# uber-research/UPSNet

Hardware: NVIDIA H100
Metric: panoptic images/sec at 1024x2048 (higher is better)
Workload: dtype bf16x3

## Files before the change

### upsnet_b200/csrc/dcn_win.cu

```cuda
#include <cuda.h>
#include <cuda_bf16.h>

#include "common.cuh"
#include "tc_ptx.cuh"
#include "tc_params.cuh"

namespace ups {

constexpr int DW_BM = 128;
constexpr int DW_WW = 32, DW_WH = 20;
constexpr int DW_PLANE = DW_WW * DW_WH * 32;
constexpr int DW_WIN_BYTES = 2 * DW_PLANE;
constexpr int DW_WIN_BUFS = 2;
constexpr int DW_KHW = 9;
constexpr int DW_GROUPS = 2;
constexpr int DW_EPI_PITCH = 36;
constexpr uint32_t DW_EPI_BYTES = DW_BM * DW_EPI_PITCH * 4;

constexpr uint32_t DW_OFF_BARS = 0;
constexpr uint32_t DW_OFF_STATS = 192;
constexpr uint32_t DW_OFF_ORG = 256;
constexpr uint32_t DW_OFF_TW = 512;
constexpr uint32_t DW_OFF_TP = DW_OFF_TW + DW_KHW * DW_BM * 16;
constexpr uint32_t DW_OFF_STAGES = DW_OFF_TP + DW_KHW * DW_BM * 4;
static_assert(DW_OFF_STAGES % 1024 == 0, "stage buffers need 1024-byte alignment (SWIZZLE_128B)");

template <int BN> struct DwCfg {
  static constexpr int NCW = BN == 128 ? 2 : 1;
  static constexpr int FRAGS = 2 / NCW;
  static constexpr int BK = BN == 128 ? 32 : 64;
  static constexpr int SPK = BK / 16;
  static constexpr int ROWB = BK * 2;
  static constexpr int CONSUMERS = 128 * NCW;
  static constexpr int WARP_TMAB = CONSUMERS / 32, WARP_TMAW = WARP_TMAB + 1, WARP_PROD0 = WARP_TMAB + 4;
  static constexpr int GROUP = 4 * (SPK / 2) * 32;
  static constexpr int PRODUCERS = GROUP * DW_GROUPS;
  static constexpr int THREADS = WARP_PROD0 * 32 + PRODUCERS;
  static constexpr int WARPGROUPS = THREADS / 128;
  static constexpr int REGS_LAUNCH = 16384 / (32 * ((THREADS / 32 + 3) / 4)) / 8 * 8;
  static constexpr int REGS_TMA = 32, REGS_CONSUMER = 128;
  static_assert(NCW * REGS_CONSUMER + REGS_TMA + (PRODUCERS / 128) * REGS_LAUNCH <= WARPGROUPS * REGS_LAUNCH,
                "setmaxnreg budgets exceed the CTA's register allocation");
  static constexpr int TABLE_IT = (DW_KHW * DW_BM + PRODUCERS - 1) / PRODUCERS;
  static constexpr uint32_t A_BYTES = 2 * DW_BM * ROWB;
  static constexpr uint32_t B_BYTES = BN * ROWB;
  static constexpr uint32_t STAGE_BYTES = 2 * B_BYTES + A_BYTES;
  static_assert(STAGE_BYTES % 1024 == 0, "stages must keep the 1024-byte alignment of the swizzled tiles");
  static constexpr int STAGES = BN == 128 ? 3 : 2;
  static_assert(STAGES <= 3, "the barrier map holds three stages");
  static constexpr uint32_t OFF_WIN = DW_OFF_STAGES + STAGES * STAGE_BYTES;
  static constexpr uint32_t OFF_EPI = OFF_WIN + DW_WIN_BUFS * DW_WIN_BYTES;
  static constexpr uint32_t SMEM = OFF_EPI + DW_EPI_BYTES + 1024;
  static_assert(SMEM <= 227 * 1024, "shared memory exceeds 227 KB");
};
template <int ROWB> __device__ __forceinline__ uint32_t dw_chunk(uint32_t j, uint32_t r) {
  return ROWB == 128 ? (j ^ (r & 7u)) : (j ^ ((r >> 1) & 3u));
}

struct DwParams {
  const void* x;
  const float* offset;
  const float* mask;
  const float* bias;
  void* y;
  int N, H, W, Cin, Cout, Cout_pad, Ho, Wo, ph, pw, dh, dw, relu, BN, tile_w, tile_h;
};

template <int BN>
__global__ void __launch_bounds__(DwCfg<BN>::THREADS, 1)
dcn_win_kernel(const __grid_constant__ CUtensorMap tm_x, const __grid_constant__ CUtensorMap tm_w, const __grid_constant__ DwParams p) {
  using C = DwCfg<BN>;
  constexpr int DW_PRODUCERS = C::PRODUCERS, DW_CONSUMERS = C::CONSUMERS;
  constexpr int DW_WARP_TMAB = C::WARP_TMAB, DW_WARP_TMAW = C::WARP_TMAW, DW_WARP_PROD0 = C::WARP_PROD0;
  constexpr int DW_BK = C::BK, SPK = C::SPK, ROWB = C::ROWB;
  extern __shared__ __align__(1024) uint8_t smem_dyn[];
  const uint32_t raw = smem_u32(smem_dyn);
  const uint32_t base = (raw + 1023u) & ~1023u;
  uint8_t* sm = smem_dyn + (base - raw);

  const int tid = threadIdx.x, warp = tid >> 5, lane = tid & 31;
  const uint32_t b_bytes = C::B_BYTES;
  const uint32_t stage_bytes = C::STAGE_BYTES;
  constexpr uint32_t NST = C::STAGES, NWB = DW_WIN_BUFS;
  const uint32_t win_base = base + C::OFF_WIN;
  float* stf = reinterpret_cast<float*>(sm + C::OFF_EPI);
  const uint32_t bar_fa = base + DW_OFF_BARS;
  const uint32_t bar_fb = bar_fa + 24;
  const uint32_t bar_em = bar_fa + 48;
  const uint32_t bar_wf = bar_fa + 104;
  const uint32_t bar_we = bar_fa + 120;
  const uint32_t bar_og = bar_fa + 136;
  int* stats = reinterpret_cast<int*>(sm + DW_OFF_STATS);
  int4* org = reinterpret_cast<int4*>(sm + DW_OFF_ORG);
  float4* tw = reinterpret_cast<float4*>(sm + DW_OFF_TW);
  int* tp = reinterpret_cast<int*>(sm + DW_OFF_TP);

  const int HoWo = p.Ho * p.Wo;
  const int nsc = p.Cin / 16;
  const int num_kb = nsc * DW_KHW / SPK;
  const int n_tiles = p.Cout_pad / BN;
  const int TW = p.tile_w, TH = p.tile_h;
  const int tw_shift = TW == 16 ? 4 : 3;
  const int tiles_w = (p.Wo + TW - 1) / TW, tiles_h = (p.Ho + TH - 1) / TH;
  const long long num_tiles = (long long)p.N * tiles_w * tiles_h * n_tiles;

  if (warp == 0) {
    if (lane == 0) {
      for (int s = 0; s < C::STAGES; ++s) {
        mbar_init(bar_fa + 8 * s, C::GROUP / 32);
        mbar_init(bar_fb + 8 * s, 1);
        mbar_init(bar_em + 8 * s, DW_CONSUMERS / 32);
      }
      for (int s = 0; s < 2; ++s) {
        mbar_init(bar_wf + 8 * s, 1);
        mbar_init(bar_we + 8 * s, DW_PRODUCERS / 32);
        mbar_init(bar_og + 8 * s, 1);
      }
      fence_mbar_init();
      for (int i = 0; i < 2; ++i) {
        stats[i * 8 + 0] = 0x7fffffff; stats[i * 8 + 1] = 0x7fffffff;
        stats[i * 8 + 2] = -0x7fffffff; stats[i * 8 + 3] = -0x7fffffff;
        stats[i * 8 + 4] = 0; stats[i * 8 + 5] = 0; stats[i * 8 + 6] = 0; stats[i * 8 + 7] = 0;
      }
    }
    __syncwarp();
  }
  if (warp == DW_WARP_TMAB && lane == 0) prefetch_tmap(&tm_w);
  if (warp == DW_WARP_TMAW && lane == 0) prefetch_tmap(&tm_x);
  __syncthreads();

  if (warp >= DW_WARP_PROD0) {
    const int pt = tid - DW_WARP_PROD0 * 32;
    const int pw = warp - DW_WARP_PROD0;
    const int group = pw / (C::GROUP / 32);
    const int u = (pw >> 2) & (SPK / 2 - 1);
    const int quad = pw & 3;
    const int r = quad * 32 + lane;
    const __nv_bfloat16* xh = reinterpret_cast<const __nv_bfloat16*>(p.x);
    uint32_t g0 = 0, wf0 = 0;
    uint32_t wf_ready = 0;
    uint32_t tile_it = 0;
    for (long long tile = blockIdx.x; tile < num_tiles; tile += gridDim.x, ++tile_it) {
      const long long mt = tile / n_tiles;
      const int tx = (int)(mt % tiles_w), ty = (int)((mt / tiles_w) % tiles_h), n = (int)(mt / ((long long)tiles_w * tiles_h));
      const int par = (int)(tile_it & 1u);
      constexpr int TIT = C::TABLE_IT;
      float4 ewv[TIT];
      int ehl[TIT], ewl[TIT];
      bool evalid[TIT];
      int mnw = 0x7fffffff, mnh = 0x7fffffff, mxw = -0x7fffffff, mxh = -0x7fffffff, sw_ = 0, sh_ = 0, cnt = 0;
#pragma unroll
      for (int it = 0; it < TIT; ++it) {
        const int e = pt + it * DW_PRODUCERS;
        ewv[it] = make_float4(0.f, 0.f, 0.f, 0.f);
        ehl[it] = 0; ewl[it] = 0; evalid[it] = false;
        if (e < DW_KHW * DW_BM) {
          const int tap = e >> 7, rr = e & 127;
          const int ry = rr >> tw_shift;
          const int wo = tx * TW + (rr & (TW - 1)), ho = ty * TH + ry;
          if (ry < TH && wo < p.Wo && ho < p.Ho) {
            const int pp = ho * p.Wo + wo;
            const int ki = tap / 3, kj = tap - ki * 3;
            const float* offp = p.offset + ((size_t)n * 2 * DW_KHW + 2 * tap) * HoWo + pp;
            const float oh = __ldg(offp), ow = __ldg(offp + HoWo);
            const float h = (float)(ho - p.ph + ki * p.dh) + oh;
            const float w = (float)(wo - p.pw + kj * p.dw) + ow;
            if (h > -1.f && w > -1.f && h < (float)p.H && w < (float)p.W) {
              const int hl = (int)floorf(h), wl = (int)floorf(w), hh = hl + 1, wh = wl + 1;
              const float lh = h - hl, lw = w - wl, ch = 1.f - lh, cw = 1.f - lw;
              const bool t_ok = hl >= 0, b_ok = hh <= p.H - 1, l_ok = wl >= 0, r_ok = wh <= p.W - 1;
              float m = 1.f;
              if (p.mask) m = __ldg(p.mask + ((size_t)n * DW_KHW + tap) * HoWo + pp);
              ewv[it].x = (t_ok && l_ok) ? ch * cw * m : 0.f;
              ewv[it].y = (t_ok && r_ok) ? ch * lw * m : 0.f;
              ewv[it].z = (b_ok && l_ok) ? lh * cw * m : 0.f;
              ewv[it].w = (b_ok && r_ok) ? lh * lw * m : 0.f;
              ehl[it] = hl; ewl[it] = wl; evalid[it] = true;
              mnw = min(mnw, wl); mxw = max(mxw, wl + 1); mnh = min(mnh, hl); mxh = max(mxh, hl + 1);
              sw_ += wl; sh_ += hl; ++cnt;
            }
          }
        }
      }
      mnw = __reduce_min_sync(0xffffffffu, mnw); mnh = __reduce_min_sync(0xffffffffu, mnh);
      mxw = __reduce_max_sync(0xffffffffu, mxw); mxh = __reduce_max_sync(0xffffffffu, mxh);
      sw_ = __reduce_add_sync(0xffffffffu, sw_); sh_ = __reduce_add_sync(0xffffffffu, sh_);
      cnt = __reduce_add_sync(0xffffffffu, cnt);
      if (lane == 0 && cnt > 0) {
        int* st = stats + par * 8;
        atomicMin(st + 0, mnw); atomicMin(st + 1, mnh); atomicMax(st + 2, mxw); atomicMax(st + 3, mxh);
        atomicAdd(st + 4, sw_); atomicAdd(st + 5, sh_); atomicAdd(st + 6, cnt);
      }
      named_bar<1, DW_PRODUCERS>();
      int ox = 0, oy = 0;
      {
        const int* st = stats + par * 8;
        const int c = st[6];
        if (c > 0) {
          const int a = st[0], b = st[1], cc = st[2], d = st[3];
          ox = (cc - a + 1 <= DW_WW) ? a : (int)floorf((float)st[4] / (float)c + 1.0f) - DW_WW / 2;
          oy = (d - b + 1 <= DW_WH) ? b : (int)floorf((float)st[5] / (float)c + 1.0f) - DW_WH / 2;
        }
      }
#pragma unroll
      for (int it = 0; it < TIT; ++it) {
        const int e = pt + it * DW_PRODUCERS;
        if (e < DW_KHW * DW_BM) {
          int code = 0;
          if (evalid[it]) {
            const int dx = ewl[it] - ox, dy = ehl[it] - oy;
            if (dx >= 0 && dx + 1 < DW_WW && dy >= 0 && dy + 1 < DW_WH) code = (dy * DW_WW + dx) * 32;
            else code = (int)(0x80000000u | ((uint32_t)(ehl[it] + 1) << 15) | (uint32_t)(ewl[it] + 1));
          }
          tw[e] = ewv[it];
          tp[e] = code;
        }
      }
      if (pt == 0) {
        org[par] = make_int4(ox, oy, n, 0);
        int* so = stats + (par ^ 1) * 8;
        so[0] = 0x7fffffff; so[1] = 0x7fffffff; so[2] = -0x7fffffff; so[3] = -0x7fffffff; so[4] = 0; so[5] = 0; so[6] = 0;
        mbar_arrive(bar_og + 8 * par);
      }
      named_bar<1, DW_PRODUCERS>();
      const __nv_bfloat16* ximg = xh + (size_t)n * p.H * p.W * (size_t)(2 * p.Cin);

      int rel = 0;
      for (int kb = (int)((uint32_t)(group - (int)g0) & 1u); kb < num_kb; kb += DW_GROUPS) {
        const uint32_t g = g0 + (uint32_t)kb;
        const uint32_t s = g % NST, it = g / NST;
        mbar_wait(bar_em + 8 * s, (it & 1u) ^ 1u);
        const uint32_t a_row = base + DW_OFF_STAGES + s * stage_bytes + 2 * b_bytes + (uint32_t)r * (uint32_t)ROWB;
#pragma unroll 1
        for (int pass = 0; pass < 4; ++pass) {
          const int sl = 2 * u + (pass >> 1), half = pass & 1;
          const int q = kb * SPK + sl;
          const int sc = q / DW_KHW, tap = q - sc * DW_KHW;
          const uint32_t wf = wf0 + (uint32_t)sc;
          if (wf >= wf_ready) {
            mbar_wait(bar_wf + 8 * (wf % NWB), (wf / NWB) & 1u);
            wf_ready = wf + 1;
          }
          const uint32_t wbuf = win_base + (wf % NWB) * (uint32_t)DW_WIN_BYTES;
          const int code = tp[tap * DW_BM + r];
          const uint32_t a_off = dw_chunk<ROWB>((uint32_t)(sl * 2 + half), (uint32_t)r) << 4;
          const float4 wv = tw[tap * DW_BM + r];
          uint4 hc[4], lc[4];
          if (code >= 0) {
            const uint32_t cl = (uint32_t)code, cr = cl + 32u;
            const uint32_t al = wbuf + cl + ((((cl >> 7) & 1u) ^ (uint32_t)half) << 4);
            const uint32_t ar = wbuf + cr + ((((cr >> 7) & 1u) ^ (uint32_t)half) << 4);
            hc[0] = lds128(al); hc[1] = lds128(ar); hc[2] = lds128(al + DW_WW * 32); hc[3] = lds128(ar + DW_WW * 32);
            lc[0] = lds128(al + DW_PLANE); lc[1] = lds128(ar + DW_PLANE);
            lc[2] = lds128(al + DW_PLANE + DW_WW * 32); lc[3] = lds128(ar + DW_PLANE + DW_WW * 32);
          } else {
            const int hl = (int)(((uint32_t)code >> 15) & 0xffffu) - 1, wl = (int)((uint32_t)code & 0x7fffu) - 1;
            const int h0 = max(hl, 0), h1 = min(hl + 1, p.H - 1), w0 = max(wl, 0), w1 = min(wl + 1, p.W - 1);
            const size_t pc = (size_t)(2 * p.Cin);
            const int cg = sc * 16 + half * 8;
            const __nv_bfloat16* b00 = ximg + ((size_t)h0 * p.W + w0) * pc + cg;
            const __nv_bfloat16* b01 = ximg + ((size_t)h0 * p.W + w1) * pc + cg;
            const __nv_bfloat16* b10 = ximg + ((size_t)h1 * p.W + w0) * pc + cg;
            const __nv_bfloat16* b11 = ximg + ((size_t)h1 * p.W + w1) * pc + cg;
            hc[0] = __ldg(reinterpret_cast<const uint4*>(b00)); lc[0] = __ldg(reinterpret_cast<const uint4*>(b00 + p.Cin));
            hc[1] = __ldg(reinterpret_cast<const uint4*>(b01)); lc[1] = __ldg(reinterpret_cast<const uint4*>(b01 + p.Cin));
            hc[2] = __ldg(reinterpret_cast<const uint4*>(b10)); lc[2] = __ldg(reinterpret_cast<const uint4*>(b10 + p.Cin));
            hc[3] = __ldg(reinterpret_cast<const uint4*>(b11)); lc[3] = __ldg(reinterpret_cast<const uint4*>(b11 + p.Cin));
          }
          uint4 ohi, olo;
          pair_blend8(wv, hc, lc, ohi, olo);
          sts128(a_row + a_off, ohi);
          sts128(a_row + DW_BM * ROWB + a_off, olo);
        }
        fence_proxy_async();
        __syncwarp();
        if (lane == 0) {
          mbar_arrive(bar_fa + 8 * s);
          while (rel < nsc && DW_KHW * (rel + 1) <= SPK * (kb + DW_GROUPS)) {
            mbar_arrive(bar_we + 8 * ((wf0 + (uint32_t)rel) % NWB));
            ++rel;
          }
        }
        rel = __shfl_sync(0xffffffffu, rel, 0);
      }
      if (lane == 0) {
        while (rel < nsc) { mbar_arrive(bar_we + 8 * ((wf0 + (uint32_t)rel) % NWB)); ++rel; }
      }
      __syncwarp();
      g0 += (uint32_t)num_kb;
      wf0 += (uint32_t)nsc;
    }
  } else if (warp >= DW_WARP_TMAB) {
    setmaxnreg_dec<C::REGS_TMA>();
    if (warp == DW_WARP_TMAW && lane == 0) {
      uint32_t wf = 0, ti = 0;
      for (long long tile = blockIdx.x; tile < num_tiles; tile += gridDim.x, ++ti) {
        const uint32_t par = ti & 1u;
        mbar_wait(bar_og + 8 * par, (ti >> 1) & 1u);
        const volatile int* ov = reinterpret_cast<const volatile int*>(&org[par]);
        const int4 o = make_int4(ov[0], ov[1], ov[2], 0);
        for (int f = 0; f < nsc; ++f, ++wf) {
          const uint32_t b = wf % NWB;
          mbar_wait(bar_we + 8 * b, ((wf / NWB) & 1u) ^ 1u);
          mbar_arrive_expect_tx(bar_wf + 8 * b, (uint32_t)DW_WIN_BYTES);
          const uint32_t dst = win_base + b * (uint32_t)DW_WIN_BYTES;
          tma_load_4d(dst, &tm_x, bar_wf + 8 * b, f * 16, o.x, o.y, o.z);
          tma_load_4d(dst + (uint32_t)DW_PLANE, &tm_x, bar_wf + 8 * b, p.Cin + f * 16, o.x, o.y, o.z);
        }
      }
    } else if (warp == DW_WARP_TMAB && lane == 0) {
      uint32_t g = 0;
      for (long long tile = blockIdx.x; tile < num_tiles; tile += gridDim.x) {
        const int n0 = (int)(tile % n_tiles) * BN;
        for (int kb = 0; kb < num_kb; ++kb, ++g) {
          const uint32_t s = g % NST, it = g / NST;
          mbar_wait(bar_em + 8 * s, (it & 1u) ^ 1u);
          const uint32_t stage = base + DW_OFF_STAGES + s * stage_bytes;
          mbar_arrive_expect_tx(bar_fb + 8 * s, 2 * b_bytes);
          tma_load_2d(stage, &tm_w, bar_fb + 8 * s, kb * DW_BK, n0);
          tma_load_2d(stage + b_bytes, &tm_w, bar_fb + 8 * s, kb * DW_BK, p.Cout_pad + n0);
        }
      }
    }
    __syncwarp();
  } else {
    setmaxnreg_inc<C::REGS_CONSUMER>();
    constexpr int FRAGS = C::FRAGS;
    const int wg = warp >> 2;
    const uint32_t dhi = ROWB == 128 ? wg_desc_hi(8 * ROWB) : wg_desc_hi_sw64(8 * ROWB);
    float d[FRAGS][BN / 2];
    constexpr uint32_t h16 = 64u * ROWB / 16u;
    __nv_bfloat16* yb = reinterpret_cast<__nv_bfloat16*>(p.y);
    uint32_t s = 0, ph = 0;
    for (long long tile = blockIdx.x; tile < num_tiles; tile += gridDim.x) {
      const long long mt = tile / n_tiles;
      const int n0 = (int)(tile % n_tiles) * BN;
      const int tx = (int)(mt % tiles_w), ty = (int)((mt / tiles_w) % tiles_h), n = (int)(mt / ((long long)tiles_w * tiles_h));
      int prev = -1;
      for (int kb = 0; kb < num_kb; ++kb) {
        mbar_wait(bar_fb + 8 * s, ph);
        mbar_wait(bar_fa + 8 * s, ph);
        const uint32_t st0 = base + DW_OFF_STAGES + s * stage_bytes;
        const uint32_t b_hi = wg_desc_lo(st0), b_lo = wg_desc_lo(st0 + b_bytes);
        const uint32_t a_hi = wg_desc_lo(st0 + 2 * b_bytes) + (uint32_t)(wg * FRAGS) * h16;
        const uint32_t a_lo = wg_desc_lo(st0 + 2 * b_bytes + DW_BM * ROWB) + (uint32_t)(wg * FRAGS) * h16;
        wgmma_fence();
#pragma unroll
        for (uint32_t k = 0; k < SPK; ++k) {
          const uint32_t acc = (kb | k) ? 1u : 0u;
          const uint64_t bh = wg_desc(b_hi + 2 * k, dhi), bl = wg_desc(b_lo + 2 * k, dhi);
#pragma unroll
          for (int f = 0; f < FRAGS; ++f) Wgmma<BN>::mma(d[f], wg_desc(a_lo + f * h16 + 2 * k, dhi), bh, acc);
#pragma unroll
          for (int f = 0; f < FRAGS; ++f) Wgmma<BN>::mma(d[f], wg_desc(a_hi + f * h16 + 2 * k, dhi), bl, 1u);
#pragma unroll
          for (int f = 0; f < FRAGS; ++f) Wgmma<BN>::mma(d[f], wg_desc(a_hi + f * h16 + 2 * k, dhi), bh, 1u);
        }
        wgmma_commit();
        wgmma_wait<1>();
#pragma unroll
        for (int f = 0; f < FRAGS; ++f) wgmma_fence_acc(d[f]);
        if (prev >= 0 && lane == 0) mbar_arrive(bar_em + 8 * prev);
        prev = (int)s;
        if (++s == NST) { s = 0; ph ^= 1u; }
      }
      wgmma_wait<0>();
#pragma unroll
      for (int f = 0; f < FRAGS; ++f) wgmma_fence_acc(d[f]);
      if (prev >= 0 && lane == 0) mbar_arrive(bar_em + 8 * prev);

      const int t = tid & 127;
      const int m = FRAGS == 2 ? t : 64 * wg + (t & 63);
      const int csub = FRAGS == 2 ? 0 : 16 * (t >> 6), cstep = FRAGS == 2 ? 16 : 32;
      const int ry = m >> tw_shift;
      const int wo = tx * TW + (m & (TW - 1)), ho = ty * TH + ry;
      const bool row_ok = ry < TH && wo < p.Wo && ho < p.Ho;
      __nv_bfloat16* yp = yb + (((size_t)n * p.Ho + ho) * p.Wo + wo) * (size_t)(2 * p.Cout);
      const uint32_t trow = smem_u32(stf + (size_t)m * DW_EPI_PITCH);
      for (int c32 = 0; c32 < BN; c32 += 32) {
        if (n0 + c32 >= p.Cout) break;
        named_bar(2 + wg, 128);
#pragma unroll
        for (int c = 0; c < BN; c += 32)
          if (c == c32) {
#pragma unroll
            for (int f = 0; f < FRAGS; ++f) acc_stage<BN, 32>(d[f], stf, DW_EPI_PITCH, 64 * (wg * FRAGS + f), c);
          }
        named_bar(2 + wg, 128);
        for (int cb = c32 + csub; cb < c32 + 32 && cb < BN; cb += cstep) {
          if (n0 + cb >= p.Cout) break;
          uint32_t rr[16];
          acc_ld16(trow + (uint32_t)(cb - c32) * 4u, rr);
          if (!row_ok) continue;
          const int co = n0 + cb;
          float o[16];
#pragma unroll
          for (int e = 0; e < 16; ++e) o[e] = __uint_as_float(rr[e]);
          if (p.bias) {
            if (co + 16 <= p.Cout) {
#pragma unroll
              for (int e4 = 0; e4 < 4; ++e4) {
                const float4 bv = __ldg(reinterpret_cast<const float4*>(p.bias + co) + e4);
                o[4 * e4] += bv.x; o[4 * e4 + 1] += bv.y; o[4 * e4 + 2] += bv.z; o[4 * e4 + 3] += bv.w;
              }
            } else {
#pragma unroll
              for (int e = 0; e < 16; ++e)
                if (co + e < p.Cout) o[e] += __ldg(p.bias + co + e);
            }
          }
          if (p.relu) {
#pragma unroll
            for (int e = 0; e < 16; ++e) o[e] = fmaxf(o[e], 0.f);
          }
          uint32_t hw[8], lw[8];
#pragma unroll
          for (int e = 0; e < 8; ++e) split_pair2(o[2 * e], o[2 * e + 1], hw[e], lw[e]);
          uint4* dh_ = reinterpret_cast<uint4*>(yp + co);
          uint4* dl_ = reinterpret_cast<uint4*>(yp + p.Cout + co);
          dh_[0] = make_uint4(hw[0], hw[1], hw[2], hw[3]); dh_[1] = make_uint4(hw[4], hw[5], hw[6], hw[7]);
          dl_[0] = make_uint4(lw[0], lw[1], lw[2], lw[3]); dl_[1] = make_uint4(lw[4], lw[5], lw[6], lw[7]);
        }
      }
    }
  }
}

__global__ void dcn_win_pack_kernel(const float* __restrict__ w, int Cout, int Cin, int Cout_pad, int K,
                                    uint16_t* __restrict__ hi, uint16_t* __restrict__ lo) {
  const size_t total = (size_t)Cout_pad * K;
  for (size_t i = (size_t)blockIdx.x * blockDim.x + threadIdx.x; i < total; i += (size_t)gridDim.x * blockDim.x) {
    const int kk = (int)(i % (size_t)K), co = (int)(i / (size_t)K);
    const int sc = kk / (16 * DW_KHW), rem = kk - sc * 16 * DW_KHW, tap = rem >> 4, c = sc * 16 + (rem & 15);
    const float v = co < Cout ? w[((size_t)co * Cin + c) * DW_KHW + tap] : 0.f;
    __nv_bfloat16 h, l;
    split_bf16(v, h, l);
    hi[i] = *reinterpret_cast<const uint16_t*>(&h);
    lo[i] = *reinterpret_cast<const uint16_t*>(&l);
  }
}

static bool dw_supported(int Cin, int Cout, int kh, int kw) {
  return kh == 3 && kw == 3 && Cin % 64 == 0 && Cin >= 64 && Cout >= 1;
}

}

extern "C" int upsnet_dcn_packed_weight_bytes(int Cout, int Cin, int kh, int kw, size_t* bytes) {
  if (!bytes || Cout <= 0 || Cin <= 0) return UPSNET_E_BADARG;
  if (!ups::dw_supported(Cin, Cout, kh, kw)) return UPSNET_E_UNSUPPORTED;
  *bytes = (size_t)2 * ups::cout_pad(Cout) * (size_t)(9 * Cin) * sizeof(uint16_t);
  return 0;
}

extern "C" int upsnet_dcn_pack_weight(const float* weight, int Cout, int Cin, int kh, int kw, void* packed, void* stream) {
  if (!weight || !packed || Cout <= 0 || Cin <= 0) return UPSNET_E_BADARG;
  if (!ups::dw_supported(Cin, Cout, kh, kw)) return UPSNET_E_UNSUPPORTED;
  const int Cout_pad = ups::cout_pad(Cout), K = 9 * Cin;
  uint16_t* hi = reinterpret_cast<uint16_t*>(packed);
  uint16_t* lo = hi + (size_t)Cout_pad * K;
  const size_t total = (size_t)Cout_pad * K;
  int blocks = (int)((total + 255) / 256);
  if (blocks > ups::kNumSMs * 16) blocks = ups::kNumSMs * 16;
  ups::dcn_win_pack_kernel<<<blocks, 256, 0, (cudaStream_t)stream>>>(weight, Cout, Cin, Cout_pad, K, hi, lo);
  UPS_CHECK_LAUNCH();
  return 0;
}

static int g_dw_force_bn = 0;

extern "C" int upsnet_dcn_set_tile_n(int bn) {
  if (bn != 0 && bn != 32 && bn != 128) return UPSNET_E_BADARG;
  g_dw_force_bn = bn;
  return 0;
}

extern "C" int upsnet_dcn_pair_forward(const void* x_pair, const float* offset, const float* mask, const void* packed,
                                       const float* bias, void* y_pair, int N, int H, int W, int Cin, int Cout, int kh,
                                       int kw, int pad_h, int pad_w, int dil_h, int dil_w, int epi_flags, void* stream) {
  using namespace ups;
  if (!x_pair || !offset || !packed || !y_pair) return UPSNET_E_BADARG;
  if (N <= 0 || H <= 0 || W <= 0 || Cin <= 0 || Cout <= 0 || pad_h < 0 || pad_w < 0 || dil_h <= 0 || dil_w <= 0) return UPSNET_E_BADARG;
  if (!dw_supported(Cin, Cout, kh, kw)) return UPSNET_E_UNSUPPORTED;
  if ((Cout % 16) != 0) return UPSNET_E_UNSUPPORTED;
  if (H >= 32767 || W >= 32767) return UPSNET_E_UNSUPPORTED;
  if ((((uintptr_t)x_pair) & 15) || (((uintptr_t)packed) & 15) || (((uintptr_t)y_pair) & 15) || (bias && (((uintptr_t)bias) & 15)))
    return UPSNET_E_UNSUPPORTED;
  DwParams p{};
  p.x = x_pair; p.offset = offset; p.mask = mask; p.bias = bias; p.y = y_pair;
  p.N = N; p.H = H; p.W = W; p.Cin = Cin; p.Cout = Cout; p.Cout_pad = cout_pad(Cout);
  p.ph = pad_h; p.pw = pad_w; p.dh = dil_h; p.dw = dil_w;
  p.Ho = conv_out_size(H, pad_h, dil_h, 3, 1);
  p.Wo = conv_out_size(W, pad_w, dil_w, 3, 1);
  if (p.Ho <= 0 || p.Wo <= 0) return UPSNET_E_BADARG;
  p.relu = (epi_flags & UPSNET_EPI_RELU) ? 1 : 0;
  const int sms = num_sms();
  p.tile_w = 16; p.tile_h = 8;
  auto dtiles = [&]() { return (long long)p.N * ((p.Wo + p.tile_w - 1) / p.tile_w) * ((p.Ho + p.tile_h - 1) / p.tile_h) * (p.Cout_pad / p.BN); };
  p.BN = 128;
  const bool wide_ok = p.Cout_pad % 128 == 0;
  const bool wide = wide_ok && (g_dw_force_bn == 128 || (g_dw_force_bn == 0 && dtiles() >= sms / 4));
  if (!wide) p.BN = 32;
  if (!wide && dtiles() < sms / 2) { p.tile_w = 8; p.tile_h = 8; }
  if (!wide && dtiles() < sms / 2) { p.tile_h = 4; }
  const long long num_tiles = dtiles();
  if (num_tiles <= 0) return 0;
  const int bk = wide ? DwCfg<128>::BK : DwCfg<32>::BK;
  const size_t smem = wide ? DwCfg<128>::SMEM : DwCfg<32>::SMEM;
  EncodeTiledFn enc = tma_encoder();
  if (!enc) return UPSNET_E_UNSUPPORTED;
  CUtensorMap tm_x, tm_w;
  {
    const cuuint64_t dx[4] = {(cuuint64_t)(2 * Cin), (cuuint64_t)W, (cuuint64_t)H, (cuuint64_t)N};
    const cuuint64_t sx[3] = {(cuuint64_t)(2 * Cin) * 2, (cuuint64_t)W * (2 * Cin) * 2, (cuuint64_t)H * W * (2 * Cin) * 2};
    const cuuint32_t bx[4] = {16, DW_WW, DW_WH, 1};
    const cuuint32_t es[4] = {1, 1, 1, 1};
    if (enc(&tm_x, CU_TENSOR_MAP_DATA_TYPE_BFLOAT16, 4, const_cast<void*>(x_pair), dx, sx, bx, es, CU_TENSOR_MAP_INTERLEAVE_NONE,
            CU_TENSOR_MAP_SWIZZLE_32B, CU_TENSOR_MAP_L2_PROMOTION_L2_128B, CU_TENSOR_MAP_FLOAT_OOB_FILL_NONE) != CUDA_SUCCESS)
      return UPSNET_E_UNSUPPORTED;
    const cuuint64_t dwt[2] = {(cuuint64_t)(9 * Cin), (cuuint64_t)(2 * p.Cout_pad)};
    const cuuint64_t sw[1] = {(cuuint64_t)(9 * Cin) * 2};
    const cuuint32_t bw[2] = {(cuuint32_t)bk, (cuuint32_t)p.BN};
    if (enc(&tm_w, CU_TENSOR_MAP_DATA_TYPE_BFLOAT16, 2, const_cast<void*>(packed), dwt, sw, bw, es, CU_TENSOR_MAP_INTERLEAVE_NONE,
            bk == 64 ? CU_TENSOR_MAP_SWIZZLE_128B : CU_TENSOR_MAP_SWIZZLE_64B, CU_TENSOR_MAP_L2_PROMOTION_L2_256B,
            CU_TENSOR_MAP_FLOAT_OOB_FILL_NONE) != CUDA_SUCCESS)
      return UPSNET_E_UNSUPPORTED;
  }
  static PerDeviceOnce configured;
  if (configured.need()) {
    UPS_CUDA(cudaFuncSetAttribute(dcn_win_kernel<32>, cudaFuncAttributeMaxDynamicSharedMemorySize, 227 * 1024));
    UPS_CUDA(cudaFuncSetAttribute(dcn_win_kernel<128>, cudaFuncAttributeMaxDynamicSharedMemorySize, 227 * 1024));
  }
  dim3 grid((unsigned)(num_tiles < sms ? num_tiles : sms));
  if (wide)
    dcn_win_kernel<128><<<grid, DwCfg<128>::THREADS, smem, (cudaStream_t)stream>>>(tm_x, tm_w, p);
  else
    dcn_win_kernel<32><<<grid, DwCfg<32>::THREADS, smem, (cudaStream_t)stream>>>(tm_x, tm_w, p);
  UPS_CHECK_LAUNCH();
  return 0;
}
```

Baseline: 129.8.

## Move deformable sample-table build to dedicated warps with double-buffered tables

Table construction (offset/mask loads, bilinear weights, window origin) moves out of the producer warps into two spare warps of the TMA warpgroup. These warps write into double-buffered shared-memory tables signalled by mbarriers, so the next tile's table is built while the current tile is gathered and multiplied. The epilogue staging buffer now reuses the idle table slot, which frees shared memory. Register budgets are rebalanced (more for TMA warps, fewer for consumers), and the producer pass loop is fully unrolled. This risks consumer register spills and adds cross-role barrier coupling.

```diff
diff --git a/upsnet_b200/csrc/dcn_win.cu b/upsnet_b200/csrc/dcn_win.cu
--- a/upsnet_b200/csrc/dcn_win.cu
+++ b/upsnet_b200/csrc/dcn_win.cu
@@ -16,13 +16,17 @@
 constexpr int DW_GROUPS = 2;
 constexpr int DW_EPI_PITCH = 36;
 constexpr uint32_t DW_EPI_BYTES = DW_BM * DW_EPI_PITCH * 4;
+constexpr int DW_TABLE_THREADS = 64;
 
 constexpr uint32_t DW_OFF_BARS = 0;
 constexpr uint32_t DW_OFF_STATS = 192;
-constexpr uint32_t DW_OFF_ORG = 256;
-constexpr uint32_t DW_OFF_TW = 512;
-constexpr uint32_t DW_OFF_TP = DW_OFF_TW + DW_KHW * DW_BM * 16;
-constexpr uint32_t DW_OFF_STAGES = DW_OFF_TP + DW_KHW * DW_BM * 4;
+constexpr uint32_t DW_OFF_ORG = 320;
+constexpr uint32_t DW_TAB_TP = DW_KHW * DW_BM * 16;
+constexpr uint32_t DW_TAB_BYTES = DW_TAB_TP + DW_KHW * DW_BM * 4;
+constexpr uint32_t DW_OFF_TAB = 512;
+constexpr uint32_t DW_OFF_STAGES = (DW_OFF_TAB + 2 * DW_TAB_BYTES + 1023) / 1024 * 1024;
+static_assert(DW_OFF_STATS + 2 * 2 * 8 * 4 <= DW_OFF_ORG && DW_OFF_ORG + 2 * 16 <= DW_OFF_TAB, "shared-memory map overlaps");
+static_assert(DW_TAB_BYTES % 16 == 0 && DW_EPI_BYTES <= DW_TAB_BYTES, "the staging buffer lives in a sample table");
 static_assert(DW_OFF_STAGES % 1024 == 0, "stage buffers need 1024-byte alignment (SWIZZLE_128B)");
 
 template <int BN> struct DwCfg {
@@ -38,10 +42,9 @@
   static constexpr int THREADS = WARP_PROD0 * 32 + PRODUCERS;
   static constexpr int WARPGROUPS = THREADS / 128;
   static constexpr int REGS_LAUNCH = 16384 / (32 * ((THREADS / 32 + 3) / 4)) / 8 * 8;
-  static constexpr int REGS_TMA = 32, REGS_CONSUMER = 128;
-  static_assert(NCW * REGS_CONSUMER + REGS_TMA + (PRODUCERS / 128) * REGS_LAUNCH <= WARPGROUPS * REGS_LAUNCH,
-                "setmaxnreg budgets exceed the CTA's register allocation");
-  static constexpr int TABLE_IT = (DW_KHW * DW_BM + PRODUCERS - 1) / PRODUCERS;
+  static constexpr int REGS_TMA = 64, REGS_CONSUMER = BN == 128 ? 112 : 96;
+  static_assert(NCW * REGS_CONSUMER + REGS_TMA + (PRODUCERS / 128) * REGS_LAUNCH == WARPGROUPS * REGS_LAUNCH,
+                "setmaxnreg budgets must add up to the CTA's register allocation");
   static constexpr uint32_t A_BYTES = 2 * DW_BM * ROWB;
   static constexpr uint32_t B_BYTES = BN * ROWB;
   static constexpr uint32_t STAGE_BYTES = 2 * B_BYTES + A_BYTES;
@@ -49,8 +52,7 @@
   static constexpr int STAGES = BN == 128 ? 3 : 2;
   static_assert(STAGES <= 3, "the barrier map holds three stages");
   static constexpr uint32_t OFF_WIN = DW_OFF_STAGES + STAGES * STAGE_BYTES;
-  static constexpr uint32_t OFF_EPI = OFF_WIN + DW_WIN_BUFS * DW_WIN_BYTES;
-  static constexpr uint32_t SMEM = OFF_EPI + DW_EPI_BYTES + 1024;
+  static constexpr uint32_t SMEM = OFF_WIN + DW_WIN_BUFS * DW_WIN_BYTES + 1024;
   static_assert(SMEM <= 227 * 1024, "shared memory exceeds 227 KB");
 };
 template <int ROWB> __device__ __forceinline__ uint32_t dw_chunk(uint32_t j, uint32_t r) {
@@ -83,17 +85,16 @@
   const uint32_t stage_bytes = C::STAGE_BYTES;
   constexpr uint32_t NST = C::STAGES, NWB = DW_WIN_BUFS;
   const uint32_t win_base = base + C::OFF_WIN;
-  float* stf = reinterpret_cast<float*>(sm + C::OFF_EPI);
   const uint32_t bar_fa = base + DW_OFF_BARS;
   const uint32_t bar_fb = bar_fa + 24;
   const uint32_t bar_em = bar_fa + 48;
   const uint32_t bar_wf = bar_fa + 104;
   const uint32_t bar_we = bar_fa + 120;
-  const uint32_t bar_og = bar_fa + 136;
+  const uint32_t bar_tf = bar_fa + 136;
+  const uint32_t bar_te = bar_fa + 152;
   int* stats = reinterpret_cast<int*>(sm + DW_OFF_STATS);
   int4* org = reinterpret_cast<int4*>(sm + DW_OFF_ORG);
-  float4* tw = reinterpret_cast<float4*>(sm + DW_OFF_TW);
-  int* tp = reinterpret_cast<int*>(sm + DW_OFF_TP);
+  uint8_t* tab = sm + DW_OFF_TAB;
 
   const int HoWo = p.Ho * p.Wo;
   const int nsc = p.Cin / 16;
@@ -114,14 +115,10 @@
       for (int s = 0; s < 2; ++s) {
         mbar_init(bar_wf + 8 * s, 1);
         mbar_init(bar_we + 8 * s, DW_PRODUCERS / 32);
-        mbar_init(bar_og + 8 * s, 1);
+        mbar_init(bar_tf + 8 * s, DW_TABLE_THREADS);
+        mbar_init(bar_te + 8 * s, DW_CONSUMERS);
       }
       fence_mbar_init();
-      for (int i = 0; i < 2; ++i) {
-        stats[i * 8 + 0] = 0x7fffffff; stats[i * 8 + 1] = 0x7fffffff;
-        stats[i * 8 + 2] = -0x7fffffff; stats[i * 8 + 3] = -0x7fffffff;
-        stats[i * 8 + 4] = 0; stats[i * 8 + 5] = 0; stats[i * 8 + 6] = 0; stats[i * 8 + 7] = 0;
-      }
     }
     __syncwarp();
   }
@@ -130,7 +127,6 @@
   __syncthreads();
 
   if (warp >= DW_WARP_PROD0) {
-    const int pt = tid - DW_WARP_PROD0 * 32;
     const int pw = warp - DW_WARP_PROD0;
     const int group = pw / (C::GROUP / 32);
     const int u = (pw >> 2) & (SPK / 2 - 1);
@@ -141,88 +137,11 @@
     uint32_t wf_ready = 0;
     uint32_t tile_it = 0;
     for (long long tile = blockIdx.x; tile < num_tiles; tile += gridDim.x, ++tile_it) {
-      const long long mt = tile / n_tiles;
-      const int tx = (int)(mt % tiles_w), ty = (int)((mt / tiles_w) % tiles_h), n = (int)(mt / ((long long)tiles_w * tiles_h));
+      const int n = (int)(tile / n_tiles / ((long long)tiles_w * tiles_h));
       const int par = (int)(tile_it & 1u);
-      constexpr int TIT = C::TABLE_IT;
-      float4 ewv[TIT];
-      int ehl[TIT], ewl[TIT];
-      bool evalid[TIT];
-      int mnw = 0x7fffffff, mnh = 0x7fffffff, mxw = -0x7fffffff, mxh = -0x7fffffff, sw_ = 0, sh_ = 0, cnt = 0;
-#pragma unroll
-      for (int it = 0; it < TIT; ++it) {
-        const int e = pt + it * DW_PRODUCERS;
-        ewv[it] = make_float4(0.f, 0.f, 0.f, 0.f);
-        ehl[it] = 0; ewl[it] = 0; evalid[it] = false;
-        if (e < DW_KHW * DW_BM) {
-          const int tap = e >> 7, rr = e & 127;
-          const int ry = rr >> tw_shift;
-          const int wo = tx * TW + (rr & (TW - 1)), ho = ty * TH + ry;
-          if (ry < TH && wo < p.Wo && ho < p.Ho) {
-            const int pp = ho * p.Wo + wo;
-            const int ki = tap / 3, kj = tap - ki * 3;
-            const float* offp = p.offset + ((size_t)n * 2 * DW_KHW + 2 * tap) * HoWo + pp;
-            const float oh = __ldg(offp), ow = __ldg(offp + HoWo);
-            const float h = (float)(ho - p.ph + ki * p.dh) + oh;
-            const float w = (float)(wo - p.pw + kj * p.dw) + ow;
-            if (h > -1.f && w > -1.f && h < (float)p.H && w < (float)p.W) {
-              const int hl = (int)floorf(h), wl = (int)floorf(w), hh = hl + 1, wh = wl + 1;
-              const float lh = h - hl, lw = w - wl, ch = 1.f - lh, cw = 1.f - lw;
-              const bool t_ok = hl >= 0, b_ok = hh <= p.H - 1, l_ok = wl >= 0, r_ok = wh <= p.W - 1;
-              float m = 1.f;
-              if (p.mask) m = __ldg(p.mask + ((size_t)n * DW_KHW + tap) * HoWo + pp);
-              ewv[it].x = (t_ok && l_ok) ? ch * cw * m : 0.f;
-              ewv[it].y = (t_ok && r_ok) ? ch * lw * m : 0.f;
-              ewv[it].z = (b_ok && l_ok) ? lh * cw * m : 0.f;
-              ewv[it].w = (b_ok && r_ok) ? lh * lw * m : 0.f;
-              ehl[it] = hl; ewl[it] = wl; evalid[it] = true;
-              mnw = min(mnw, wl); mxw = max(mxw, wl + 1); mnh = min(mnh, hl); mxh = max(mxh, hl + 1);
-              sw_ += wl; sh_ += hl; ++cnt;
-            }
-          }
-        }
-      }
-      mnw = __reduce_min_sync(0xffffffffu, mnw); mnh = __reduce_min_sync(0xffffffffu, mnh);
-      mxw = __reduce_max_sync(0xffffffffu, mxw); mxh = __reduce_max_sync(0xffffffffu, mxh);
-      sw_ = __reduce_add_sync(0xffffffffu, sw_); sh_ = __reduce_add_sync(0xffffffffu, sh_);
-      cnt = __reduce_add_sync(0xffffffffu, cnt);
-      if (lane == 0 && cnt > 0) {
-        int* st = stats + par * 8;
-        atomicMin(st + 0, mnw); atomicMin(st + 1, mnh); atomicMax(st + 2, mxw); atomicMax(st + 3, mxh);
-        atomicAdd(st + 4, sw_); atomicAdd(st + 5, sh_); atomicAdd(st + 6, cnt);
-      }
-      named_bar<1, DW_PRODUCERS>();
-      int ox = 0, oy = 0;
-      {
-        const int* st = stats + par * 8;
-        const int c = st[6];
-        if (c > 0) {
-          const int a = st[0], b = st[1], cc = st[2], d = st[3];
-          ox = (cc - a + 1 <= DW_WW) ? a : (int)floorf((float)st[4] / (float)c + 1.0f) - DW_WW / 2;
-          oy = (d - b + 1 <= DW_WH) ? b : (int)floorf((float)st[5] / (float)c + 1.0f) - DW_WH / 2;
-        }
-      }
-#pragma unroll
-      for (int it = 0; it < TIT; ++it) {
-        const int e = pt + it * DW_PRODUCERS;
-        if (e < DW_KHW * DW_BM) {
-          int code = 0;
-          if (evalid[it]) {
-            const int dx = ewl[it] - ox, dy = ehl[it] - oy;
-            if (dx >= 0 && dx + 1 < DW_WW && dy >= 0 && dy + 1 < DW_WH) code = (dy * DW_WW + dx) * 32;
-            else code = (int)(0x80000000u | ((uint32_t)(ehl[it] + 1) << 15) | (uint32_t)(ewl[it] + 1));
-          }
-          tw[e] = ewv[it];
-          tp[e] = code;
-        }
-      }
-      if (pt == 0) {
-        org[par] = make_int4(ox, oy, n, 0);
-        int* so = stats + (par ^ 1) * 8;
-        so[0] = 0x7fffffff; so[1] = 0x7fffffff; so[2] = -0x7fffffff; so[3] = -0x7fffffff; so[4] = 0; so[5] = 0; so[6] = 0;
-        mbar_arrive(bar_og + 8 * par);
-      }
-      named_bar<1, DW_PRODUCERS>();
+      mbar_wait(bar_tf + 8 * par, (tile_it >> 1) & 1u);
+      const float4* tw = reinterpret_cast<const float4*>(tab + par * DW_TAB_BYTES);
+      const int* tp = reinterpret_cast<const int*>(tab + par * DW_TAB_BYTES + DW_TAB_TP);
       const __nv_bfloat16* ximg = xh + (size_t)n * p.H * p.W * (size_t)(2 * p.Cin);
 
       int rel = 0;
@@ -231,7 +150,7 @@
         const uint32_t s = g % NST, it = g / NST;
         mbar_wait(bar_em + 8 * s, (it & 1u) ^ 1u);
         const uint32_t a_row = base + DW_OFF_STAGES + s * stage_bytes + 2 * b_bytes + (uint32_t)r * (uint32_t)ROWB;
-#pragma unroll 1
+#pragma unroll
         for (int pass = 0; pass < 4; ++pass) {
           const int sl = 2 * u + (pass >> 1), half = pass & 1;
           const int q = kb * SPK + sl;
@@ -292,11 +211,80 @@
     }
   } else if (warp >= DW_WARP_TMAB) {
     setmaxnreg_dec<C::REGS_TMA>();
-    if (warp == DW_WARP_TMAW && lane == 0) {
+    if (warp >= DW_WARP_TMAB + 2) {
+      const int lt = tid - (DW_WARP_TMAB + 2) * 32, tw_w = warp - (DW_WARP_TMAB + 2);
+      uint32_t ti = 0;
+      for (long long tile = blockIdx.x; tile < num_tiles; tile += gridDim.x, ++ti) {
+        const long long mt = tile / n_tiles;
+        const int tx = (int)(mt % tiles_w), ty = (int)((mt / tiles_w) % tiles_h), n = (int)(mt / ((long long)tiles_w * tiles_h));
+        const uint32_t par = ti & 1u;
+        mbar_wait(bar_te + 8 * par, ((ti >> 1) & 1u) ^ 1u);
+        float4* tw = reinterpret_cast<float4*>(tab + par * DW_TAB_BYTES);
+        int* tp = reinterpret_cast<int*>(tab + par * DW_TAB_BYTES + DW_TAB_TP);
+        int mnw = 0x7fffffff, mnh = 0x7fffffff, mxw = -0x7fffffff, mxh = -0x7fffffff, sw_ = 0, sh_ = 0, cnt = 0;
+#pragma unroll 2
+        for (int e = lt; e < DW_KHW * DW_BM; e += DW_TABLE_THREADS) {
+          float4 wv = make_float4(0.f, 0.f, 0.f, 0.f);
+          int code = 0;
+          const int tap = e >> 7, rr = e & 127;
+          const int ry = rr >> tw_shift;
+          const int wo = tx * TW + (rr & (TW - 1)), ho = ty * TH + ry;
+          if (ry < TH && wo < p.Wo && ho < p.Ho) {
+            const int pp = ho * p.Wo + wo;
+            const int ki = tap / 3, kj = tap - ki * 3;
+            const float* offp = p.offset + ((size_t)n * 2 * DW_KHW + 2 * tap) * HoWo + pp;
+            const float oh = __ldg(offp), ow = __ldg(offp + HoWo);
+            const float m = p.mask ? __ldg(p.mask + ((size_t)n * DW_KHW + tap) * HoWo + pp) : 1.f;
+            const float h = (float)(ho - p.ph + ki * p.dh) + oh;
+            const float w = (float)(wo - p.pw + kj * p.dw) + ow;
+            if (h > -1.f && w > -1.f && h < (float)p.H && w < (float)p.W) {
+              const int hl = (int)floorf(h), wl = (int)floorf(w), hh = hl + 1, wh = wl + 1;
+              const float lh = h - hl, lw = w - wl, ch = 1.f - lh, cw = 1.f - lw;
+              const bool t_ok = hl >= 0, b_ok = hh <= p.H - 1, l_ok = wl >= 0, r_ok = wh <= p.W - 1;
+              wv.x = (t_ok && l_ok) ? ch * cw * m : 0.f;
+              wv.y = (t_ok && r_ok) ? ch * lw * m : 0.f;
+              wv.z = (b_ok && l_ok) ? lh * cw * m : 0.f;
+              wv.w = (b_ok && r_ok) ? lh * lw * m : 0.f;
+              code = (int)(0x80000000u | ((uint32_t)(hl + 1) << 15) | (uint32_t)(wl + 1));
+              mnw = min(mnw, wl); mxw = max(mxw, wl + 1); mnh = min(mnh, hl); mxh = max(mxh, hl + 1);
+              sw_ += wl; sh_ += hl; ++cnt;
+            }
+          }
+          tw[e] = wv;
+          tp[e] = code;
+        }
+        int* st = stats + (par * 2 + tw_w) * 8;
+        mnw = __reduce_min_sync(0xffffffffu, mnw); mnh = __reduce_min_sync(0xffffffffu, mnh);
+        mxw = __reduce_max_sync(0xffffffffu, mxw); mxh = __reduce_max_sync(0xffffffffu, mxh);
+        sw_ = __reduce_add_sync(0xffffffffu, sw_); sh_ = __reduce_add_sync(0xffffffffu, sh_);
+        cnt = __reduce_add_sync(0xffffffffu, cnt);
+        if (lane == 0) { st[0] = mnw; st[1] = mnh; st[2] = mxw; st[3] = mxh; st[4] = sw_; st[5] = sh_; st[6] = cnt; }
+        named_bar<4, DW_TABLE_THREADS>();
+        const int* s0 = stats + par * 2 * 8;
+        const int* s1 = s0 + 8;
+        const int c = s0[6] + s1[6];
+        int ox = 0, oy = 0;
+        if (c > 0) {
+          const int a = min(s0[0], s1[0]), b = min(s0[1], s1[1]), cc = max(s0[2], s1[2]), d = max(s0[3], s1[3]);
+          ox = (cc - a + 1 <= DW_WW) ? a : (int)floorf((float)(s0[4] + s1[4]) / (float)c + 1.0f) - DW_WW / 2;
+          oy = (d - b + 1 <= DW_WH) ? b : (int)floorf((float)(s0[5] + s1[5]) / (float)c + 1.0f) - DW_WH / 2;
+        }
+        for (int e = lt; e < DW_KHW * DW_BM; e += DW_TABLE_THREADS) {
+          const int code = tp[e];
+          if (code < 0) {
+            const int hl = (int)(((uint32_t)code >> 15) & 0xffffu) - 1, wl = (int)((uint32_t)code & 0x7fffu) - 1;
+            const int dx = wl - ox, dy = hl - oy;
+            if (dx >= 0 && dx + 1 < DW_WW && dy >= 0 && dy + 1 < DW_WH) tp[e] = (dy * DW_WW + dx) * 32;
+          }
+        }
+        if (lt == 0) org[par] = make_int4(ox, oy, n, 0);
+        mbar_arrive(bar_tf + 8 * par);
+      }
+    } else if (warp == DW_WARP_TMAW && lane == 0) {
       uint32_t wf = 0, ti = 0;
       for (long long tile = blockIdx.x; tile < num_tiles; tile += gridDim.x, ++ti) {
         const uint32_t par = ti & 1u;
-        mbar_wait(bar_og + 8 * par, (ti >> 1) & 1u);
+        mbar_wait(bar_tf + 8 * par, (ti >> 1) & 1u);
         const volatile int* ov = reinterpret_cast<const volatile int*>(&org[par]);
         const int4 o = make_int4(ov[0], ov[1], ov[2], 0);
         for (int f = 0; f < nsc; ++f, ++wf) {
@@ -331,8 +319,8 @@
     float d[FRAGS][BN / 2];
     constexpr uint32_t h16 = 64u * ROWB / 16u;
     __nv_bfloat16* yb = reinterpret_cast<__nv_bfloat16*>(p.y);
-    uint32_t s = 0, ph = 0;
-    for (long long tile = blockIdx.x; tile < num_tiles; tile += gridDim.x) {
+    uint32_t s = 0, ph = 0, ti = 0;
+    for (long long tile = blockIdx.x; tile < num_tiles; tile += gridDim.x, ++ti) {
       const long long mt = tile / n_tiles;
       const int n0 = (int)(tile % n_tiles) * BN;
       const int tx = (int)(mt % tiles_w), ty = (int)((mt / tiles_w) % tiles_h), n = (int)(mt / ((long long)tiles_w * tiles_h));
@@ -376,6 +364,7 @@
       const int wo = tx * TW + (m & (TW - 1)), ho = ty * TH + ry;
       const bool row_ok = ry < TH && wo < p.Wo && ho < p.Ho;
       __nv_bfloat16* yp = yb + (((size_t)n * p.Ho + ho) * p.Wo + wo) * (size_t)(2 * p.Cout);
+      float* stf = reinterpret_cast<float*>(tab + (ti & 1u) * DW_TAB_BYTES);
       const uint32_t trow = smem_u32(stf + (size_t)m * DW_EPI_PITCH);
       for (int c32 = 0; c32 < BN; c32 += 32) {
         if (n0 + c32 >= p.Cout) break;
@@ -422,6 +411,7 @@
           dl_[0] = make_uint4(lw[0], lw[1], lw[2], lw[3]); dl_[1] = make_uint4(lw[4], lw[5], lw[6], lw[7]);
         }
       }
+      mbar_arrive(bar_te + 8 * (ti & 1u));
     }
   }
 }
```

Result: no change. 130.2 (median of 6 runs) (+0.3%).
